# lschoenm/MerKurio

Measured on AMD Instinct MI355X. Metric: Gbases/s scanned (150bp FASTQ, 10k 31-mers); % HBM roofline at 1/2/4/8 GPUs, higher is better.
Workload: dtype u8

## Files before the change

### include/merkurio_hip.h

```cpp
#ifndef MERKURIO_HIP_H
#define MERKURIO_HIP_H

#include <stddef.h>
#include <stdint.h>

#ifdef __cplusplus
extern "C" {
#endif

#define MK_ABI_VERSION 7

#define MK_OK 0
#define MK_E_EMPTY_PATTERN (-1)
#define MK_E_INVALID_Q (-2)
#define MK_E_PATTERN_TOO_LONG (-3)
#define MK_E_NO_PATTERNS (-4)
#define MK_E_NOMEM (-5)
#define MK_E_PAIR_MISMATCH (-6)
#define MK_E_HIP (-7)
#define MK_E_CAPACITY (-8)
#define MK_E_INVALID_ARG (-9)
#define MK_E_UNSUPPORTED (-10)
#define MK_E_RCCL (-11)
#define MK_E_CORRUPT (-12)
// ... 82 lines not shown
#define MK_SUM_RECORDS 2
#define MK_SUM_BASES 3
#define MK_SUM_CANDIDATES 4

int mk_scan_device(mk_matcher *m, const void *d_seq, uint64_t n_bytes, const void *d_seq_off, uint64_t n_rec,
                   uint32_t mode, void *d_rec_flags, void *d_hits, uint64_t hits_cap, void *d_n_hits,
                   void *d_counters, void *stream);

int mk_matcher_check_device(mk_matcher *m, void *stream);

int mk_matcher_hint_hit_density(mk_matcher *m, uint32_t records_hit_per_1000);

int mk_matcher_set_fixed_record_length(mk_matcher *m, uint32_t record_length);

int mk_matcher_hint_record_lengths(mk_matcher *m, int equal_lengths);

int mk_order_hits(const mk_matcher *m, mk_hit *hits, uint64_t n_hits);
int mk_order_hits_device(mk_matcher *m, void *d_hits, uint64_t n_hits, void *stream);
int mk_matcher_order_info(const mk_matcher *m, uint32_t *path, uint32_t *n_bins, uint32_t *max_bin);
int mk_matcher_order_stats(const mk_matcher *m, uint64_t calls[4]);

const char *mk_matcher_kernel_name(const mk_matcher *m);
int mk_matcher_launch_info(const mk_matcher *m, uint32_t *grid_blocks, uint32_t *block_threads, uint32_t *lds_bytes);
int mk_matcher_enable_timing(mk_matcher *m, uint32_t slots);
int mk_matcher_kernel_times(mk_matcher *m, float *ms, uint32_t cap, uint32_t *n_out);

int mk_extract_single(mk_matcher *m, const uint8_t *seq, const uint64_t *off, uint64_t n_rec, int logging,
                      int invert, uint8_t *keep, mk_row *rows, uint64_t rows_cap, uint64_t *n_rows,
                      mk_counters *counters, uint32_t *pattern_hit_counts);
int mk_extract_paired(mk_matcher *m, const uint8_t *seq1, const uint64_t *off1, uint64_t n_rec1,
                      const uint8_t *seq2, const uint64_t *off2, uint64_t n_rec2, int logging, int invert,
                      uint8_t *keep, mk_row *rows, uint64_t rows_cap, uint64_t *n_rows, mk_counters *counters,
                      uint32_t *pattern_hit_counts);
int mk_tag_records(mk_matcher *m, const uint8_t *seq, const uint64_t *off, uint64_t n_rec, int logging,
                   int filter_matching, int invert, uint8_t *keep, mk_row *rows, uint64_t rows_cap, uint64_t *n_rows,
                   mk_counters *counters, uint32_t *pattern_hit_counts, uint64_t *found_off, uint32_t *found_pat,
                   uint64_t found_cap);
int mk_extract_fastq_text(mk_matcher *m, const uint8_t *text, uint64_t n_text, int logging, int invert, uint64_t rec_cap,
                          uint64_t *n_rec, uint64_t *rec_start, uint8_t *keep, mk_row *rows, uint64_t rows_cap, uint64_t *n_rows,
                          mk_counters *counters, uint32_t *pattern_hit_counts, uint32_t *status);
int mk_upload_text_ahead(mk_matcher *m, const uint8_t *text, uint64_t n_text);
int mk_host_alloc(size_t bytes, void **out);
void mk_host_free(void *p);
int mk_matcher_batch_times(const mk_matcher *m, float ms[4]);

int mk_tag_value(const mk_matcher *m, const uint32_t *found_pat, uint64_t n_found, const char *existing, char *out,
// ... 209 lines not shown
```

### merkurio_amd/csrc/matcher.cpp

```cpp
#include <hip/hip_runtime.h>

#include <algorithm>
#include <chrono>
#include <cmath>
#include <cstdarg>
#include <cstdio>
#include <cstdlib>
#include <cstring>
#include <memory>
#include <string>
#include <vector>

#include "host_common.h"
#include "matcher_internal.h"
#include "scan_kernel.h"

namespace mk {

thread_local char g_last_error[512] = "";

int fail(int code, const char *fmt, ...) {
    va_list ap;
    va_start(ap, fmt);
    vsnprintf(g_last_error, sizeof(g_last_error), fmt, ap);
// ... 461 lines not shown
int mk_matcher_filter_info(const mk_matcher *m, uint32_t *q_gram, uint32_t *stride, uint64_t *entries,
                           uint64_t *table_bytes) {
    if (!m) return fail(MK_E_INVALID_ARG, "null matcher");
    if (q_gram) *q_gram = m->q;
    if (stride) *stride = m->S;
    if (entries) *entries = m->entries;
    if (table_bytes) *table_bytes = (uint64_t)m->table_slots * sizeof(TableEntry);
    return MK_OK;
}

int mk_matcher_class_info(const mk_matcher *m, uint32_t *split_len, uint32_t *n_short, uint32_t *q_gram2, uint32_t *stride2) {
    if (!m) return fail(MK_E_INVALID_ARG, "null matcher");
    if (split_len) *split_len = m->split_len;
    if (n_short) *n_short = m->n_short;
    if (q_gram2) *q_gram2 = m->q2;
    if (stride2) *stride2 = m->S2;
    return MK_OK;
}

int mk_matcher_filter_mode(const mk_matcher *m, uint32_t *in_lds, uint64_t *filter_bytes) {
    if (!m) return fail(MK_E_INVALID_ARG, "null matcher");
    if (in_lds) *in_lds = m->gbloom_blocks ? 0 : 1;
    if (filter_bytes) *filter_bytes = m->gbloom_blocks ? (uint64_t)m->gbloom_blocks * 8 : (uint64_t)kBloomBytes;
    return MK_OK;
}

int mk_scan_device(mk_matcher *m, const void *d_seq, uint64_t n_bytes, const void *d_seq_off, uint64_t n_rec,
                   uint32_t mode, void *d_rec_flags, void *d_hits, uint64_t hits_cap, void *d_n_hits,
                   void *d_counters, void *stream) {
    if (!m) return fail(MK_E_INVALID_ARG, "null matcher");
    if (mode > MK_MODE_HITS) return fail(MK_E_INVALID_ARG, "unknown mode %u", mode);
    if (((uintptr_t)d_seq & 15) != 0) return fail(MK_E_INVALID_ARG, "d_seq must be 16-byte aligned");
    if (((uintptr_t)d_rec_flags & 3) != 0) return fail(MK_E_INVALID_ARG, "d_rec_flags must be 4-byte aligned");
    const uint32_t rec_len = m->batch_rec_len ? m->batch_rec_len : m->fixed_rec_len;
    if (rec_len && n_bytes != n_rec * (uint64_t)rec_len)
        return fail(MK_E_INVALID_ARG, "fixed record length %u: %llu records are not %llu bytes", rec_len, (unsigned long long)n_rec,
                    (unsigned long long)n_bytes);
    if (!d_n_hits || !d_rec_flags || (!d_seq_off && n_rec && !rec_len)) return fail(MK_E_INVALID_ARG, "null device buffer");
    if (mode == MK_MODE_HITS && !d_hits && hits_cap) return fail(MK_E_INVALID_ARG, "d_hits is null");
    hipStream_t st = (hipStream_t)stream;
    MK_HIP(hipSetDevice(m->device));
    launch_clear((uint32_t *)d_rec_flags, (n_rec + 3) / 4, (unsigned long long *)d_n_hits, st);
    MK_HIP(hipGetLastError());
    if (mode == MK_MODE_HITS) MK_HIP(hipMemsetAsync(m->d_error, 0, sizeof(uint32_t), st));
    m->last_n_rec = n_rec;
    if (n_rec == 0 || n_bytes == 0) return MK_OK;
// ... 14 lines not shown
    p.n_pat = m->n_pat;
    p.q = m->q;
    const uint64_t kmask = m->q >= 32 ? ~0ull : ((1ull << (2 * m->q)) - 1);
    p.key_mask_lo = (uint32_t)kmask;
    p.key_mask_hi = (uint32_t)(kmask >> 32);
    p.case_insensitive = (m->flags & MK_FLAG_ASCII_CASE_INSENSITIVE) ? 1 : 0;
    p.s2 = m->split_len ? m->S2 : 0;
    p.s2_log2 = m->S2 >= 8 ? 3 : m->S2 >= 4 ? 2 : m->S2 >= 2 ? 1 : 0;
    p.key2_mask = (1u << (2 * m->q2)) - 1u;
    p.short_bytes = m->q2 <= kShortByteMaxQ;
    p.short_bitmap = m->d_short_table;
    p.uniform_len = m->uniform_len;
    p.rec_flags32 = (uint32_t *)d_rec_flags;
    p.hits = (mk_hit *)d_hits;
    p.hits_cap = (mode == MK_MODE_HITS) ? hits_cap : 0;
    p.n_hits = (unsigned long long *)d_n_hits;
    p.counters = (unsigned long long *)d_counters;
    p.error_word = m->d_error;
    const uint64_t waves_per_block = kBlockThreads / 64;
    uint64_t blocks = (n_tiles + waves_per_block - 1) / waves_per_block;
    if (blocks > (uint64_t)m->num_cus) blocks = m->num_cus;
    p.stage = m->d_stage;
    p.rec_per_byte = (double)n_rec / (double)n_bytes;
    const uint64_t tiles_per_wave = n_tiles / (blocks * waves_per_block);
    p.tile_run = m->tile_run ? m->tile_run : tiles_per_wave >= 16 ? 4 : tiles_per_wave >= 8 ? 2 : 1;
    p.rec_index = nullptr;
    p.rec_len = rec_len;
    p.inv_rec_len = rec_len ? 1.0 / (double)rec_len : 0.0;
    if (m->ragged && !rec_len && n_rec < (1ull << 32)) {
        int rc_i = ensure((void **)&m->d_rec_index, &m->d_rec_index_cap, ((n_bytes >> kRecIndexShift) + 2) * sizeof(uint32_t));
        if (rc_i) return rc_i;
        launch_rec_index(p.rec_off, n_rec, n_bytes, m->d_rec_index, st);
        p.rec_index = m->d_rec_index;
    }
    const size_t slots = m->ev_start.size();
    const size_t slot = slots ? (size_t)(m->timed_launches % slots) : 0;
    if (slots) MK_HIP(hipEventRecord(m->ev_start[slot], st));
    const uint32_t kDensePerMille = mode == MK_MODE_HITS ? 95 : 145;
    const bool plain_loads = m->hit_density_pm >= kDensePerMille && !m->split_len;
    const int flavour = plain_loads ? 0 : 1;
    const bool listed = !(plain_loads && m->gbloom_blocks == 0) && mode != MK_MODE_HITS && n_rec < (1ull << 32);
    p.flag_list = listed ? m->d_flag_list : nullptr;
    p.flag_counts = m->d_flag_counts;
    p.flag_cap = kFlagListCap;
    const char *name = launch_scan(p, (int)m->S, m->q > 16, mode == MK_MODE_HITS, m->gbloom_blocks != 0, flavour, (int)blocks, st);
    if (!name) return fail(MK_E_UNSUPPORTED, "no kernel for stride %u", m->S);
    if (slots) {
        MK_HIP(hipEventRecord(m->ev_stop[slot], st));
        m->timed_launches++;
    }
    if (listed)
        launch_flag_scatter(m->d_flag_list, m->d_flag_counts, kFlagListCap, (uint32_t)(blocks * waves_per_block), (uint8_t *)d_rec_flags, st);
    if (d_counters) {
        launch_count_flags(p, st);
        if (mode == MK_MODE_HITS && p.hits && p.hits_cap) launch_hist_hits(p, m->num_cus, st);
    }
    m->kernel_name = name;
    m->last_grid = (int)blocks;
    MK_HIP(hipGetLastError());
    return MK_OK;
}

static int take_device_errors(mk_matcher *m, hipStream_t st) {
    uint32_t w = 0;
    MK_HIP(hipMemcpyAsync(&w, m->d_error, sizeof(w), hipMemcpyDeviceToHost, st));
    MK_HIP(hipStreamSynchronize(st));
    if (!w) return MK_OK;
    MK_HIP(hipMemsetAsync(m->d_error, 0, sizeof(w), st));
    return fail(MK_E_UNSUPPORTED, "an occurrence lies 4 GiB or more into its record: a single record must be shorter than 4 GiB "
                                  "(mk_hit.pos is 32 bits); the tuples of that scan are not usable");
}

int mk_matcher_check_device(mk_matcher *m, void *stream) {
    if (!m) return fail(MK_E_INVALID_ARG, "null matcher");
    MK_HIP(hipSetDevice(m->device));
    return take_device_errors(m, (hipStream_t)stream);
}

int mk_matcher_hint_hit_density(mk_matcher *m, uint32_t records_hit_per_1000) {
    if (!m) return fail(MK_E_INVALID_ARG, "null matcher");
    m->hit_density_pm = records_hit_per_1000 > 1000 ? 1000 : records_hit_per_1000;
// ... 379 lines not shown
```

### merkurio_amd/csrc/matcher_internal.h

```cpp
#pragma once
#include <hip/hip_runtime.h>

#include <mutex>
#include <vector>

#include "filter.hpp"
#include "scan_kernel.h"
#include "host_common.h"

struct mk_matcher {
    int device = 0;
    int num_cus = 256;
    uint32_t algo = MK_ALGO_AC;
    uint32_t flags = 0;
    uint32_t n_pat = 0;
    std::vector<uint8_t> pat_bytes;
    std::vector<uint32_t> pat_off;
    uint32_t uniform_len = 0;
    uint32_t q = 0, S = 1;
    uint32_t split_len = 0, S2 = 0, q2 = 0, n_short = 0;
    uint32_t *d_short_table = nullptr;
    uint64_t entries = 0;
    uint32_t table_slots = 0;
    uint32_t *d_bloom = nullptr;
    uint32_t gbloom_blocks = 0;
    uint32_t tile_run = 0;
    uint32_t hit_density_pm = 0;
    bool ragged = false;
    uint32_t fixed_rec_len = 0, batch_rec_len = 0;
    uint32_t *d_rec_index = nullptr;
// ... 32 lines not shown
        size_t d_text_cap = 0, d_ing_a_cap = 0, d_ing_b_cap = 0, d_fa_seq_cap = 0;
    } txt[2];
    uint32_t bam_piece = 0;
    uint8_t *d_flags2 = nullptr;
    size_t d_flags2_cap = 0;
    void *d_refs = nullptr;
    size_t d_refs_cap = 0;
    std::vector<uint8_t> refs_names;
    std::vector<uint64_t> refs_off;
    uint32_t refs_slots = 0;
    bool refs_valid = false;
    struct AheadSlot {
        void *d = nullptr;
        size_t cap = 0;
        hipEvent_t ev = nullptr;
        const uint8_t *text = nullptr;
        uint64_t n = 0;
    } ahead[4];
    hipStream_t stream_ahead = nullptr;
    std::mutex ahead_mu;
    float batch_ms[4] = {0, 0, 0, 0};
    const char *kernel_name = "";
    int last_grid = 0;
    std::vector<hipEvent_t> ev_start, ev_stop;
    uint64_t timed_launches = 0;
    void *comm = nullptr;
    int comm_rank = 0, comm_size = 0;
};

namespace mk {
int ensure_device(void **p, size_t *cap, size_t need);
extern thread_local double g_alloc_ms, g_free_ms;
int batch_check(const uint8_t *seq_bytes, const uint64_t *seq_off, uint64_t n_rec, uint64_t *n_bytes);
int batch_upload(mk_matcher *m, const uint8_t *seq_bytes, const uint64_t *seq_off, uint64_t n_rec, uint64_t n_bytes, uint32_t *batch_len);
int batch_scan(mk_matcher *m, uint64_t n_bytes, uint64_t n_rec, uint32_t mode, uint32_t batch_len, uint64_t cap, uint64_t limit,
               unsigned long long *found);
int batch_flags(mk_matcher *m, uint64_t n_rec, uint8_t *rec_flags, uint64_t *flagged_out);
int order_hits_on_device(mk_matcher *m, void *d_hits, uint64_t n_hits, bool ac_order, uint64_t rec_bound, void *stream);
int hip_fail(hipError_t e, const char *what);
}
```

### merkurio_amd/csrc/scan_kernel.h

```cpp
#pragma once
#include <hip/hip_runtime.h>
#include <stdint.h>

#include "../../include/merkurio_hip.h"
#include "filter.hpp"

namespace mk {

constexpr uint32_t kHitStage = 1024;
constexpr uint32_t kFlagListCap = 2048;

struct ScanParams {
    const uint8_t *seq;
    uint64_t n_bytes;
    const uint64_t *rec_off;
    uint64_t n_rec;
    const uint32_t *bloom;
    uint32_t gbloom_blocks;
    const TableEntry *table;
    uint32_t table_mask;
    const uint8_t *pat_bytes;
    const uint32_t *pat_off;
    uint32_t n_pat;
    uint32_t q;
    uint32_t key_mask_lo;
    uint32_t key_mask_hi;
    uint32_t s2;
    uint32_t s2_log2;
    uint32_t key2_mask;
    uint32_t short_bytes;
    const uint32_t *short_bitmap;
    uint32_t case_insensitive;
    uint32_t uniform_len;
    double rec_per_byte;
    uint32_t tile_run;
    const uint32_t *rec_index;
    uint32_t rec_len;
    double inv_rec_len;
    mk_hit *stage;
    uint32_t *rec_flags32;
    uint32_t *flag_list;
    uint32_t *flag_counts;
    uint32_t flag_cap;
    mk_hit *hits;
    uint64_t hits_cap;
    unsigned long long *n_hits;
    unsigned long long *counters;
    uint32_t *error_word;
};

const char *launch_scan(const ScanParams &p, int S, bool wide, bool emit, bool global_filter, int flavour, int grid_blocks,
                        hipStream_t stream);

template <int S, int QC, bool EMIT, bool GF, int FL, int MC = 0>
void launch_variant(const ScanParams &p, int grid_blocks, hipStream_t stream);

uint32_t scan_lds_bytes();

// ... 130 lines not shown
```

### merkurio_amd/csrc/scan_kernel_impl.hpp

```cpp
#pragma once
#include <algorithm>

#include "scan_kernel.h"

namespace mk {

typedef uint32_t u32x4 __attribute__((ext_vector_type(4)));

__device__ __forceinline__ uint32_t pack4_top(uint32_t d) { return (d & 0x06060606u) * 0x00820820u; }
__device__ __forceinline__ uint32_t pack16(uint4 v) {
    const uint32_t u0 = pack4_top(v.x), u1 = pack4_top(v.y), u2 = pack4_top(v.z), u3 = pack4_top(v.w);
    const uint32_t lo16 = __builtin_amdgcn_perm(u1, u0, 0x0c0c0703u);
    const uint32_t hi16 = __builtin_amdgcn_perm(u3, u2, 0x07030c0cu);
    return lo16 | hi16;
}

__device__ __forceinline__ uint4 load16(const uint8_t *__restrict__ seq, uint64_t pos, uint64_t n) {
    if (pos + 16 <= n) return *reinterpret_cast<const uint4 *>(seq + pos);
    uint32_t w[4] = {0, 0, 0, 0};
    if (pos < n) {
        uint32_t rem = (uint32_t)(n - pos);
        for (uint32_t i = 0; i < rem; ++i) w[i >> 2] |= (uint32_t)seq[pos + i] << (8 * (i & 3));
    }
    return make_uint4(w[0], w[1], w[2], w[3]);
// ... 352 lines not shown
    if constexpr (!GF) {
        const uint4 *src = reinterpret_cast<const uint4 *>(P.bloom);
        uint4 *dst = reinterpret_cast<uint4 *>(bloom);
        for (uint32_t i = threadIdx.x; i < kBloomWords / 4; i += kBlockThreads) dst[i] = src[i];
    }
    if constexpr (MC != 0) {
        const uint4 *src2 = reinterpret_cast<const uint4 *>(P.short_bitmap);
        uint4 *dst2 = reinterpret_cast<uint4 *>(lds_all);
        for (uint32_t i = threadIdx.x; i < kShortBitmapWords / 4; i += kBlockThreads) dst2[i] = src2[i];
    }
    if constexpr (!GF || MC != 0) __syncthreads();
    const uint2 *__restrict__ gbloom = reinterpret_cast<const uint2 *>(P.bloom);
    const uint32_t gmask = P.gbloom_blocks;

    if (P.counters && blockIdx.x == 0 && threadIdx.x == 0) {
        atomicAdd(&P.counters[P.n_pat + MK_SUM_RECORDS], (unsigned long long)P.n_rec);
        atomicAdd(&P.counters[P.n_pat + MK_SUM_BASES], (unsigned long long)P.n_bytes);
    }
    const uint32_t lane = threadIdx.x & 63u;
    const uint32_t wave_in_block = __builtin_amdgcn_readfirstlane(threadIdx.x >> 6);
    const uint64_t wave_id = (uint64_t)blockIdx.x * (kBlockThreads / 64) + wave_in_block;
    const uint64_t n_waves = (uint64_t)gridDim.x * (kBlockThreads / 64);
    constexpr int NS = G::kNS;
    constexpr uint64_t kTileBytes = (uint64_t)kTileChunks * kChunkBytes;
    const uint32_t mask_lo = P.key_mask_lo, mask_hi = P.key_mask_hi;
    const uint8_t *__restrict__ seq = P.seq;
    const uint64_t n_bytes = P.n_bytes;
    CandEntry *ring = reinterpret_cast<CandEntry *>(bloom + kBloomWords) + wave_in_block * kRingEntries;
    uint32_t *ctx_ring = bloom + wave_in_block * kRingEntries;
    uint32_t q_head = 0, q_count = 0, n_cand = 0;
    HitRing hr;
    hr.q = reinterpret_cast<uint2 *>(bloom + kBloomWords + (kBlockThreads / 64) * kRingEntries * 2) + wave_in_block * kHitSlots;
    hr.count = 0;
    hr.stage = EMIT ? P.stage + wave_id * (uint64_t)kHitStage : nullptr;
    hr.staged = 0;
    hr.flist = (!kWide && !EMIT && P.flag_list) ? P.flag_list + wave_id * (uint64_t)P.flag_cap : nullptr;
    hr.nflag = 0;
    uint32_t n_true = 0;
    uint32_t abl_acc = 0;

    auto halo = [&](uint32_t pk_cur, uint32_t pk_nxt, uint32_t &w1, uint32_t &w2) __attribute__((always_inline)) {
        w1 = 0;
        w2 = 0;
        if constexpr (G::kNeedW1) {
            const uint32_t n0 = __builtin_amdgcn_readlane(pk_nxt, 0);
            w1 = __builtin_amdgcn_update_dpp(n0, pk_cur, 0x130, 0xf, 0xf, false);
        }
// ... 140 lines not shown
                    const uint32_t khi = __builtin_amdgcn_alignbit(w2, w1, sh) & mask_hi;
                    const uint32_t t = __builtin_amdgcn_alignbit(khi, klo, 24);
                    slot_h = __umul24(klo, 0x9E3779u) + __umul24(t, 0x85EBCBu) + (t & 0xFF000000u);
                }
                if constexpr (kCtx) {
                    const uint32_t pb = 2u * j * S;
                    const uint32_t prev7 = pb >= 14u ? (w0 >> (pb - 14u)) : __builtin_amdgcn_alignbit(w0, wm1, (pb + 18u) & 31u);
                    const uint32_t next7 = stream32_rt(w0, w1, w2, pb + 2u * (uint32_t)QC);
                    slot_c = (prev7 & 0x3FFFu) | ((next7 & 0x3FFFu) << 14);
                }
                slot_t = t_base + j * S;
                if constexpr (MC != 0) {
                    const uint32_t j2 = (j - 16u) << P.s2_log2;
                    const uint32_t fp2 = short_fp(__builtin_amdgcn_alignbit(w1, w0, 2u * j2) & P.key2_mask);
                    const bool is2 = j >= 16u;
                    slot_h = is2 ? fp2 : main_fp(slot_h);
                    slot_t = is2 ? t_base + j2 : slot_t;
                }
                slot_full = true;
            }
        } while (__ballot(cand != 0));
    };

    const uint64_t n_main_tiles = n_bytes >= kChunkBytes ? (n_bytes - kChunkBytes) / kTileBytes : 0;
    if (wave_id * (P.tile_run ? P.tile_run : 1u) < n_main_tiles) {
        const uint32_t run = P.tile_run ? P.tile_run : 1u;
        const uint64_t jump = (n_waves - 1) * (uint64_t)run + 1;
        uint64_t ld_tile = wave_id * run;
        uint32_t ld_run = 0;
        uint32_t ld_g = 0;
        const uint64_t last_tile = n_main_tiles - 1;
        const uint8_t *ld_ptr = seq + (ld_tile < last_tile ? ld_tile : last_tile) * kTileBytes + lane * 16;
        auto nt_load = [](const uint8_t *p) -> uint4 {
            if constexpr (NTL) {
                const u32x4 nv = __builtin_nontemporal_load(reinterpret_cast<const u32x4 *>(p));
                return make_uint4(nv.x, nv.y, nv.z, nv.w);
            } else {
                return *reinterpret_cast<const uint4 *>(p);
            }
        };
        auto load_group = [&](uint4 &a, uint4 &b, uint4 &c, uint4 &d) __attribute__((always_inline)) {
            a = nt_load(ld_ptr);
            b = nt_load(ld_ptr + kChunkBytes);
            c = nt_load(ld_ptr + 2 * kChunkBytes);
            d = nt_load(ld_ptr + 3 * kChunkBytes);
            ld_ptr += 4 * kChunkBytes;
            if (++ld_g == (uint32_t)(kTileChunks + 1) / 4) {
                ld_g = 0;
                if (++ld_run == run) {
                    ld_run = 0;
                    ld_tile += jump;
                } else {
                    ld_tile += 1;
                }
                const uint64_t t = ld_tile < last_tile ? ld_tile : last_tile;
                ld_ptr = seq + t * kTileBytes + lane * 16;
            }
        };
        uint4 r0, r1, r2, r3;
        load_group(r0, r1, r2, r3);
        uint32_t pk_prev = 0;
        uint32_t pk_pp = 0, pk_tile_prev = 0;
        bool pd_on = false;
        uint32_t pd_h0 = 0, pd_h1 = 0, pd_cur = 0, pd_nxt = 0, pd_wm1 = 0;
        uint2 pd_b0 = make_uint2(0, 0), pd_b1 = pd_b0;
        uint64_t pd_cpos = 0;
        auto test_pending = [&]() __attribute__((always_inline)) {
            auto pass = [](uint32_t h, uint2 blk) -> uint32_t {
                const uint32_t hb = gbloom_bits(h);
                return (blk.x >> (hb >> 27)) & (blk.x >> (hb >> 12)) & (blk.y >> (hb >> 22)) & (blk.y >> (hb >> 17)) & 1u;
            };
            uint32_t cand = pass(pd_h0, pd_b0);
            if constexpr (NS > 1) cand |= pass(pd_h1, pd_b1) << 1;
            if (__ballot(cand != 0)) queue_candidates(pd_cur, pd_nxt, pd_wm1, cand, pd_cpos, pd_h0, pd_h1);
        };
        uint64_t last_push_base = 0;
        uint32_t sc_run = 0;
        for (uint64_t tile = wave_id * run; tile < n_main_tiles;) {
            const uint64_t base = tile * kTileBytes;
            if constexpr (kCtx) {
                pk_tile_prev = 0;
                if (base >= 16) pk_tile_prev = pack16(*reinterpret_cast<const uint4 *>(seq + base - 16));
            }
            if (base - last_push_base >= (1ull << 30)) {
                last_push_base = base;
                flush_slots();
                if (hr.count) drain_hits<EMIT, FL>(P, hr, newest_end, lane, n_true);
                if (q_count && !pend_on) issue_probe(q_count < 64 ? q_count : 64);
            }
#pragma unroll 1
            for (int g = 0; g < (kTileChunks + 1) / 4; ++g) {
                const uint32_t p0 = pack16(r0), p1 = pack16(r1), p2 = pack16(r2), p3 = pack16(r3);
                asm volatile("" ::"v"(p0), "v"(p1), "v"(p2), "v"(p3) : "memory");
                if (pend_on) consume_probe();
                load_group(r0, r1, r2, r3);
                {
                    uint32_t q0 = p0, q1 = p1, q2 = p2;
#pragma unroll 1
                    for (int k = 0; k < 4; ++k) {
                        const int ci = 4 * g + k - 1;
                        if constexpr (kPipe) {
                            uint32_t nh0 = 0, nh1 = 0, nwm1 = 0;
                            uint2 nb0 = make_uint2(0, 0), nb1 = nb0;
                            if (ci >= 0) {
                                uint32_t w1, w2;
                                halo(pk_prev, q0, w1, w2);
                                nh0 = sample_hash<S, QC>(pk_prev, w1, w2, 0, mask_lo, mask_hi);
                                nb0 = gbloom[gbloom_block(nh0, gmask)];
                                if constexpr (NS > 1) {
                                    nh1 = sample_hash<S, QC>(pk_prev, w1, w2, 2 * S, mask_lo, mask_hi);
                                    nb1 = gbloom[gbloom_block(nh1, gmask)];
                                }
                                nwm1 = __builtin_amdgcn_update_dpp(__builtin_amdgcn_readlane(pk_pp, 63), pk_prev, 0x138, 0xf, 0xf, false);
                            }
// ... 18 lines not shown
                                queue_candidates(pk_prev, q0, wm1, ck, base + (uint64_t)ci * kChunkBytes, h0, h1);
                            }
                        }
                        if constexpr (kCtx) pk_pp = ci < 0 ? pk_tile_prev : pk_prev;
                        pk_prev = q0;
                        q0 = q1;
                        q1 = q2;
                        q2 = p3;
                    }
                }
                if constexpr ((MK_ABLATE & 8) != 0) {
                    if (q_count >= MK_ISSUE_AT) {
                        q_head = (q_head + q_count) & (kRingEntries - 1);
                        q_count = 0;
                    }
                } else if (!pend_on && q_count >= (FL == 0 ? MK_ISSUE_AT_DENSE : MK_ISSUE_AT)) {
                    issue_probe(q_count < 64 ? q_count : 64);
                }
                if constexpr (FL == 0 && MK_DRAIN_AT_DENSE <= 64) {
                    if (hr.count >= MK_DRAIN_AT_DENSE) drain_hits<EMIT, FL>(P, hr, newest_end, lane, n_true);
                }
                pk_prev = p3;
            }
            if (++sc_run == run) {
                sc_run = 0;
                tile += jump;
            } else {
                tile += 1;
            }
        }
        if constexpr (kPipe) {
            if (pd_on) test_pending();
        }
    }
    if (pend_on) consume_probe();

    {
        const uint64_t tail_rank = (wave_id + n_waves - (n_main_tiles / (P.tile_run ? P.tile_run : 1u)) % n_waves) % n_waves;
        for (uint64_t cpos = n_main_tiles * kTileBytes + tail_rank * kChunkBytes; cpos < n_bytes; cpos += n_waves * kChunkBytes) {
            const uint32_t pk_cur = pack16(load16(seq, cpos + lane * 16, n_bytes));
            const uint32_t pk_nxt = pack16(load16(seq, cpos + kChunkBytes + lane * 16, n_bytes));
            uint32_t h0 = 0, h1 = 0;
            const uint32_t ck = filter_chunk(pk_cur, pk_nxt, h0, h1);
            if constexpr ((MK_ABLATE & 4) != 0) n_cand += ck;
            if (__ballot(ck != 0)) {
                uint32_t wm1 = 0;
                if constexpr (kCtx) {
                    const uint64_t mine = cpos + lane * 16;
                    if (mine >= 16) wm1 = pack16(load16(seq, mine - 16, n_bytes));
                }
                queue_candidates(pk_cur, pk_nxt, wm1, ck, cpos, h0, h1);
            }
        }
    }

    flush_slots();
    while (q_count) drain_ring(q_count < 64 ? q_count : 64);
    if (hr.count) drain_hits<EMIT, FL>(P, hr, newest_end, lane, n_true);
    if constexpr (EMIT) flush_stage<!kWide>(P, hr, lane);
    if (hr.flist && lane == 0) P.flag_counts[wave_id] = hr.nflag;
    if ((MK_ABLATE & 1) != 0 && abl_acc == 0xFFFFFFFFu) n_cand++;
    if (P.counters) {
// ... 13 lines not shown
```

### merkurio_amd/native.py

```python
import ctypes as C
import time
import importlib.util
import os

import numpy as np

from . import build as _build

MK_OK = 0
MK_E_EMPTY_PATTERN = -1
MK_E_INVALID_Q = -2
MK_E_PATTERN_TOO_LONG = -3
MK_E_NO_PATTERNS = -4
MK_E_NOMEM = -5
MK_E_PAIR_MISMATCH = -6
MK_E_HIP = -7
MK_E_CAPACITY = -8
MK_E_INVALID_ARG = -9
MK_E_UNSUPPORTED = -10
MK_E_RCCL = -11
MK_E_CORRUPT = -12
MK_COMM_ID_BYTES = 128

MK_ALGO_AUTO, MK_ALGO_AC, MK_ALGO_BNDMQ = 0, 1, 2
MK_FLAG_ASCII_CASE_INSENSITIVE = 1
MK_MODE_ANY, MK_MODE_HITS = 0, 1
MK_NUM_SUMMARY = 8
MK_SUM_HITS, MK_SUM_RECORDS_HIT, MK_SUM_RECORDS, MK_SUM_BASES, MK_SUM_CANDIDATES = 0, 1, 2, 3, 4

HIT_DTYPE = np.dtype([("rec", "<u8"), ("pat", "<u4"), ("pos", "<u4")])
ROW_DTYPE = np.dtype([("rec", "<u8"), ("pat", "<u4"), ("pos", "<u4"), ("file", "<u4"), ("_pad", "<u4")])

EXPORTS = [
    "mk_abi_version", "mk_last_error", "mk_device_count", "mk_read_kmers_from_text", "mk_parse_pattern_list",
    "mk_reverse_complement", "mk_canonical", "mk_recommend_aho_corasick", "mk_tune_q_value", "mk_generate_masks",
    "mk_free", "mk_matcher_create", "mk_matcher_create_ex", "mk_plan_geometry", "mk_matcher_destroy", "mk_matcher_algo", "mk_matcher_num_patterns",
    "mk_matcher_filter_info", "mk_matcher_class_info", "mk_matcher_filter_mode", "mk_scan_batch", "mk_scan_device", "mk_order_hits", "mk_order_hits_device", "mk_matcher_order_info", "mk_matcher_order_stats", "mk_matcher_kernel_name",
    "mk_matcher_launch_info", "mk_matcher_enable_timing", "mk_matcher_kernel_times", "mk_matcher_hint_hit_density", "mk_matcher_hint_record_lengths", "mk_matcher_set_fixed_record_length", "mk_matcher_check_device",
    "mk_extract_single", "mk_extract_fastq_text", "mk_upload_text_ahead", "mk_host_alloc", "mk_host_free", "mk_extract_paired", "mk_tag_records", "mk_tag_value", "mk_matcher_batch_times", "mk_synth_reads_device",
    "mk_synth_reads_host", "mk_synth_reads_device_range", "mk_reduce_counters", "mk_reduce_prepare", "mk_comm_available", "mk_comm_unique_id", "mk_comm_init",
    "mk_comm_reduce_counters", "mk_comm_size", "mk_comm_destroy",
    "mk_codec_create", "mk_codec_destroy", "mk_bgzf_deflate_bound", "mk_bgzf_deflate", "mk_bgzf_deflate_pieces", "mk_bgzf_inflate", "mk_bgzf_members", "mk_bgzf_eof",
    "mk_codec_times", "mk_codec_set_pass_limits", "mk_codec_set_inflate_kernel", "mk_codec_set_gzip_chunk", "mk_gzip_inflate_device", "mk_gzip_text_read", "mk_gzip_text_device", "mk_gzip_text_release", "mk_gzip_info", "mk_extract_fastq_bgzf", "mk_extract_window",
    "mk_tag_bam_window", "mk_matcher_set_bam_piece", "mk_tag_sam_window", "mk_tag_sam_bam_window", "mk_tag_bam_sam_window",
]


class MerkurioError(RuntimeError):
    def __init__(self, code, msg):
        super().__init__(f"[{code}] {msg}")
        self.code = code


class PatternError(MerkurioError):
    KINDS = {MK_E_EMPTY_PATTERN: "EmptyPattern", MK_E_INVALID_Q: "InvalidQGramLength",
             MK_E_PATTERN_TOO_LONG: "PatternTooLong"}

    @property
    def kind(self):
        return self.KINDS.get(self.code, "?")


class MatcherOptions(C.Structure):
    _fields_ = [("struct_size", C.c_uint32), ("force_stride", C.c_uint32), ("force_global_filter", C.c_uint32),
                ("gbloom_log2_blocks", C.c_uint32), ("tile_run", C.c_uint32), ("gbloom_kib", C.c_uint32),
                ("length_classes", C.c_uint32), ("force_split_len", C.c_uint32), ("force_stride2", C.c_uint32),
                ("force_q2", C.c_uint32)]

    def __init__(self, force_stride=0, force_global_filter=False, gbloom_log2_blocks=0, tile_run=0, gbloom_kib=0,
                 length_classes=0, force_split_len=0, force_stride2=0, force_q2=0, force_single_class=False):
        super().__init__(C.sizeof(MatcherOptions), int(force_stride), int(bool(force_global_filter)),
                         int(gbloom_log2_blocks), int(tile_run), int(gbloom_kib),
                         1 if force_single_class else int(length_classes), int(force_split_len), int(force_stride2), int(force_q2))


class WindowText(C.Structure):
    _fields_ = [("text", C.c_void_p), ("text_cap", C.c_uint64), ("tail", C.c_void_p), ("tail_cap", C.c_uint64), ("kept", C.c_void_p),
                ("kept_cap", C.c_uint64), ("n_text", C.c_uint64), ("n_used", C.c_uint64), ("n_tail", C.c_uint64), ("n_kept_bytes", C.c_uint64)]


class WindowSource(C.Structure):
    _fields_ = [("head", C.c_void_p), ("n_head", C.c_uint64), ("text", C.c_void_p), ("n_text", C.c_uint64), ("bgzf", C.c_void_p),
                ("n_bgzf", C.c_uint64), ("members", C.c_void_p), ("n_members", C.c_uint64), ("device_text", C.c_void_p), ("n_device_text", C.c_uint64), ("ends_at_record", C.c_uint32),
                ("reserved", C.c_uint32), ("rec_start", C.c_void_p), ("tail", C.c_void_p), ("tail_cap", C.c_uint64), ("kept", C.c_void_p),
                ("kept_cap", C.c_uint64), ("all", C.c_void_p), ("all_cap", C.c_uint64), ("n_window", C.c_uint64), ("n_used", C.c_uint64),
                ("n_tail", C.c_uint64), ("n_kept_bytes", C.c_uint64), ("n_rec_seen", C.c_uint64)]


MK_TEXT_FASTQ, MK_TEXT_FASTA = 0, 1


class BamWindow(C.Structure):
    _fields_ = [("head", C.c_void_p), ("n_head", C.c_uint64), ("bgzf", C.c_void_p), ("n_bgzf", C.c_uint64), ("members", C.c_void_p), ("n_members", C.c_uint64),
                ("last", C.c_uint32), ("filter_matching", C.c_uint32), ("invert", C.c_uint32), ("tag", C.c_uint8 * 2), ("reserved", C.c_uint8 * 2),
                ("block_bytes", C.c_uint32), ("tail", C.c_void_p), ("tail_cap", C.c_uint64), ("out", C.c_void_p), ("out_cap", C.c_uint64),
                ("rows", C.c_void_p), ("rows_cap", C.c_uint64), ("row_name", C.c_void_p), ("names", C.c_void_p), ("names_cap", C.c_uint64),
# ... 90 lines not shown
    L.mk_matcher_num_patterns.argtypes = [C.c_void_p]
    L.mk_matcher_num_patterns.restype = C.c_uint32
    L.mk_matcher_create.argtypes = [C.c_void_p, C.c_void_p, C.c_uint32, C.c_uint32, C.c_uint32, C.c_uint32, C.c_int32,
                                    C.POINTER(C.c_void_p)]
    L.mk_matcher_create_ex.argtypes = [C.c_void_p, C.c_void_p, C.c_uint32, C.c_uint32, C.c_uint32, C.c_uint32, C.c_int32,
                                       C.POINTER(MatcherOptions), C.POINTER(C.c_void_p)]
    L.mk_synth_reads_device_range.argtypes = [C.c_void_p, C.c_uint64, C.c_uint64, C.c_uint64, C.c_uint32, C.c_uint32,
                                              C.c_void_p, C.c_void_p, C.c_void_p]
    L.mk_reduce_counters.argtypes = [C.POINTER(C.c_void_p), C.c_int, C.POINTER(C.c_void_p), C.c_size_t, C.c_void_p]
    L.mk_reduce_prepare.argtypes = [C.POINTER(C.c_void_p), C.c_int]
    L.mk_comm_unique_id.argtypes = [C.c_void_p]
    L.mk_comm_init.argtypes = [C.c_void_p, C.c_void_p, C.c_int, C.c_int]
    L.mk_comm_reduce_counters.argtypes = [C.c_void_p, C.c_void_p, C.c_size_t, C.c_void_p]
    L.mk_comm_destroy.argtypes = [C.c_void_p]
    L.mk_comm_size.argtypes = [C.c_void_p, C.POINTER(C.c_int)]
    L.mk_scan_batch.argtypes = [C.c_void_p, C.c_void_p, C.c_void_p, C.c_uint64, C.c_uint32, C.c_void_p, C.c_void_p,
                                C.c_uint64, C.POINTER(C.c_uint64)]
    L.mk_scan_device.argtypes = [C.c_void_p, C.c_void_p, C.c_uint64, C.c_void_p, C.c_uint64, C.c_uint32, C.c_void_p,
                                 C.c_void_p, C.c_uint64, C.c_void_p, C.c_void_p, C.c_void_p]
    L.mk_order_hits.argtypes = [C.c_void_p, C.c_void_p, C.c_uint64]
    L.mk_order_hits_device.argtypes = [C.c_void_p, C.c_void_p, C.c_uint64, C.c_void_p]
    L.mk_matcher_order_info.argtypes = [C.c_void_p, C.POINTER(C.c_uint32), C.POINTER(C.c_uint32), C.POINTER(C.c_uint32)]
    L.mk_matcher_launch_info.argtypes = [C.c_void_p, C.POINTER(C.c_uint32), C.POINTER(C.c_uint32), C.POINTER(C.c_uint32)]
    L.mk_matcher_enable_timing.argtypes = [C.c_void_p, C.c_uint32]
    L.mk_matcher_hint_hit_density.argtypes = [C.c_void_p, C.c_uint32]
    L.mk_matcher_hint_record_lengths.argtypes = [C.c_void_p, C.c_int]
    L.mk_matcher_set_fixed_record_length.argtypes = [C.c_void_p, C.c_uint32]
    L.mk_matcher_check_device.argtypes = [C.c_void_p, C.c_void_p]
    L.mk_matcher_batch_times.argtypes = [C.c_void_p, C.POINTER(C.c_float)]
    L.mk_matcher_kernel_times.argtypes = [C.c_void_p, C.c_void_p, C.c_uint32, C.POINTER(C.c_uint32)]
    L.mk_matcher_filter_info.argtypes = [C.c_void_p, C.POINTER(C.c_uint32), C.POINTER(C.c_uint32),
                                         C.POINTER(C.c_uint64), C.POINTER(C.c_uint64)]
    L.mk_matcher_filter_mode.argtypes = [C.c_void_p, C.POINTER(C.c_uint32), C.POINTER(C.c_uint64)]
    L.mk_plan_geometry.argtypes = [C.c_void_p, C.c_uint32, C.POINTER(MatcherOptions)] + [C.POINTER(C.c_uint32)] * 7
    L.mk_matcher_class_info.argtypes = [C.c_void_p, C.POINTER(C.c_uint32), C.POINTER(C.c_uint32), C.POINTER(C.c_uint32),
                                        C.POINTER(C.c_uint32)]
    L.mk_extract_single.argtypes = [C.c_void_p, C.c_void_p, C.c_void_p, C.c_uint64, C.c_int, C.c_int, C.c_void_p,
                                    C.c_void_p, C.c_uint64, C.POINTER(C.c_uint64), C.POINTER(Counters), C.c_void_p]
    L.mk_extract_fastq_text.argtypes = [C.c_void_p, C.c_void_p, C.c_uint64, C.c_int, C.c_int, C.c_uint64, C.POINTER(C.c_uint64), C.c_void_p,
                                        C.c_void_p, C.c_void_p, C.c_uint64, C.POINTER(C.c_uint64), C.POINTER(Counters), C.c_void_p,
                                        C.POINTER(C.c_uint32)]
    L.mk_upload_text_ahead.argtypes = [C.c_void_p, C.c_void_p, C.c_uint64]
    L.mk_host_alloc.argtypes = [C.c_size_t, C.POINTER(C.c_void_p)]
    L.mk_host_free.argtypes = [C.c_void_p]
    L.mk_host_free.restype = None
    L.mk_codec_create.argtypes = [C.c_int, C.POINTER(C.c_void_p)]
# ... 142 lines not shown
    q = load().mk_tune_q_value(len(pattern))
    if q == 0:
        raise MerkurioError(MK_E_PATTERN_TOO_LONG, "Pattern length is too long for BNDMq.")
    return q


def generate_masks(pattern: bytes):
    src = np.frombuffer(bytes(pattern) + b"\0", dtype=np.uint8)
    masks = np.zeros(256, dtype=np.uint64)
    accept = C.c_uint64()
    _check(load().mk_generate_masks(src.ctypes.data, len(pattern), masks.ctypes.data, C.byref(accept)))
    return masks.tolist(), accept.value


def plan_geometry(lengths, options=None):
    lens = np.ascontiguousarray(lengths, dtype=np.uint32)
    opt = None if options is None else (options if isinstance(options, MatcherOptions) else MatcherOptions(**options))
    v = [C.c_uint32() for _ in range(7)]
    _check(load().mk_plan_geometry(lens.ctypes.data, len(lens), None if opt is None else C.byref(opt), *[C.byref(x) for x in v]))
    keys = ("q_gram", "stride", "in_lds", "split_len", "n_short", "q_gram2", "stride2")
    return dict(zip(keys, (x.value for x in v)))


class Matcher:

    def __init__(self, patterns, algo=MK_ALGO_AUTO, q=0, case_insensitive=False, device=0, options=None):
        self.patterns = [p.encode() if isinstance(p, str) else bytes(p) for p in patterns]
        data, off = pack_list(self.patterns)
        self._h = C.c_void_p()
        flags = MK_FLAG_ASCII_CASE_INSENSITIVE if case_insensitive else 0
        if options is None:
            _check(load().mk_matcher_create(data.ctypes.data, off.ctypes.data, len(self.patterns), algo, q, flags,
                                            device, C.byref(self._h)))
        else:
            opt = options if isinstance(options, MatcherOptions) else MatcherOptions(**options)
            _check(load().mk_matcher_create_ex(data.ctypes.data, off.ctypes.data, len(self.patterns), algo, q, flags,
                                               device, C.byref(opt), C.byref(self._h)))
        self.device = device

    def close(self):
        if getattr(self, "_h", None):
            load().mk_matcher_destroy(self._h)
            self._h = None

    def __del__(self):
        try:
# ... 1 lines not shown
        except Exception:
            pass

    @property
    def handle(self):
        return self._h

    @property
    def algo(self):
        return load().mk_matcher_algo(self._h)

    @property
    def use_ac(self):
        return self.algo == MK_ALGO_AC

    @property
    def kernel_name(self):
        return load().mk_matcher_kernel_name(self._h).decode()

    def launch_info(self):
        g, b, l = C.c_uint32(), C.c_uint32(), C.c_uint32()
        _check(load().mk_matcher_launch_info(self._h, C.byref(g), C.byref(b), C.byref(l)))
        return {"grid_blocks": g.value, "block_threads": b.value, "lds_bytes": l.value}

    def batch_times_ms(self):
        ms = (C.c_float * 4)()
        _check(load().mk_matcher_batch_times(self._h, ms))
        return {"upload": ms[0], "device": ms[1], "download": ms[2], "host": ms[3]}

    def order_info(self):
        a, b, c = C.c_uint32(), C.c_uint32(), C.c_uint32()
        _check(load().mk_matcher_order_info(self._h, C.byref(a), C.byref(b), C.byref(c)))
        return {"path": a.value, "bins": b.value, "max_bin": c.value}

    def enable_timing(self, slots):
        _check(load().mk_matcher_enable_timing(self._h, slots))
        self._timing_slots = slots

    def kernel_times_ms(self):
        cap = max(1, getattr(self, "_timing_slots", 0))
        ms = np.zeros(cap, dtype=np.float32)
        n = C.c_uint32()
        _check(load().mk_matcher_kernel_times(self._h, ms.ctypes.data, cap, C.byref(n)))
        return ms[:n.value].tolist()

    def filter_info(self):
# ... 508 lines not shown
```

Before: 6217.

## Replace tile runs with long contiguous tiles and balanced short-tile remainder geometry

Each wave now scans one long contiguous tile per run, merged from several short tiles so the overlap chunk is not reloaded, instead of a sequence of separate adjacent tiles. The remaining bytes are split into short tiles whose size is chosen to balance loads across waves. The old run-jump bookkeeping in the loader and scan loops is removed and a run of 8 is added for large inputs. This reduces redundant halo loads and tail imbalance, at the cost of per-tile base and group computation, possibly fewer blocks, and a new geometry-inspection API.

```diff
diff --git a/include/merkurio_hip.h b/include/merkurio_hip.h
--- a/include/merkurio_hip.h
+++ b/include/merkurio_hip.h
@@ -128,6 +128,17 @@
 
 const char *mk_matcher_kernel_name(const mk_matcher *m);
 int mk_matcher_launch_info(const mk_matcher *m, uint32_t *grid_blocks, uint32_t *block_threads, uint32_t *lds_bytes);
+typedef struct {
+    uint64_t n_waves;
+    uint64_t n_long_tiles, long_tile_bytes;
+    uint64_t n_short_tiles, short_tile_bytes;
+    uint64_t tail_start;
+    uint32_t long_tile_loads, short_tile_loads;
+    uint32_t tile_run;
+    uint32_t reserved;
+} mk_tile_geometry;
+int mk_scan_tile_geometry(uint64_t n_bytes, uint64_t n_waves, uint32_t tile_run, mk_tile_geometry *out);
+int mk_matcher_scan_geometry(const mk_matcher *m, mk_tile_geometry *out);
 int mk_matcher_enable_timing(mk_matcher *m, uint32_t slots);
 int mk_matcher_kernel_times(mk_matcher *m, float *ms, uint32_t cap, uint32_t *n_out);
 
diff --git a/merkurio_amd/csrc/matcher.cpp b/merkurio_amd/csrc/matcher.cpp
--- a/merkurio_amd/csrc/matcher.cpp
+++ b/merkurio_amd/csrc/matcher.cpp
@@ -507,6 +507,34 @@
     if (!m) return fail(MK_E_INVALID_ARG, "null matcher");
     if (in_lds) *in_lds = m->gbloom_blocks ? 0 : 1;
     if (filter_bytes) *filter_bytes = m->gbloom_blocks ? (uint64_t)m->gbloom_blocks * 8 : (uint64_t)kBloomBytes;
+    return MK_OK;
+}
+
+static void export_geometry(const TileGeometry &g, uint64_t n_waves, uint32_t run, mk_tile_geometry *out) {
+    out->n_waves = n_waves;
+    out->n_long_tiles = g.n_long;
+    out->long_tile_bytes = g.long_bytes;
+    out->n_short_tiles = g.n_short;
+    out->short_tile_bytes = g.short_bytes;
+    out->tail_start = g.tail_start;
+    out->long_tile_loads = g.long_loads;
+    out->short_tile_loads = g.short_loads;
+    out->tile_run = run;
+    out->reserved = 0;
+}
+
+int mk_scan_tile_geometry(uint64_t n_bytes, uint64_t n_waves, uint32_t tile_run, mk_tile_geometry *out) {
+    if (!out) return fail(MK_E_INVALID_ARG, "null geometry");
+    if (n_waves == 0 || tile_run > kMaxTileRun)
+        return fail(MK_E_INVALID_ARG, "tile geometry: %llu waves, tile_run %u (0..8)", (unsigned long long)n_waves, tile_run);
+    if (tile_run == 0) tile_run = tile_run_rule(n_bytes, n_waves);
+    export_geometry(tile_geometry(n_bytes, n_waves, tile_run), n_waves, tile_run, out);
+    return MK_OK;
+}
+
+int mk_matcher_scan_geometry(const mk_matcher *m, mk_tile_geometry *out) {
+    if (!m || !out) return fail(MK_E_INVALID_ARG, "null argument");
+    export_geometry(m->last_geo, (uint64_t)m->last_grid * (kBlockThreads / 64), m->last_run, out);
     return MK_OK;
 }
 
@@ -567,8 +595,18 @@
     if (blocks > (uint64_t)m->num_cus) blocks = m->num_cus;
     p.stage = m->d_stage;
     p.rec_per_byte = (double)n_rec / (double)n_bytes;
-    const uint64_t tiles_per_wave = n_tiles / (blocks * waves_per_block);
-    p.tile_run = m->tile_run ? m->tile_run : tiles_per_wave >= 16 ? 4 : tiles_per_wave >= 8 ? 2 : 1;
+    uint32_t run = m->tile_run ? m->tile_run : tile_run_rule(n_bytes, blocks * waves_per_block);
+    while (run > 1 && blocks * waves_per_block * ((uint64_t)(run * (kTileChunks + 1) - 1) * kChunkBytes) > (1ull << 30)) --run;
+    if (run > 1 && blocks < (uint64_t)m->num_cus) {
+        const uint64_t long_bytes = (uint64_t)(run * (kTileChunks + 1) - 1) * kChunkBytes;
+        blocks = std::min<uint64_t>(blocks, std::max<uint64_t>(1, n_bytes / (long_bytes * waves_per_block)));
+    }
+    const TileGeometry geo = tile_geometry(n_bytes, blocks * waves_per_block, run);
+    p.n_long_tiles = geo.n_long;
+    p.n_tiles = geo.n_long + geo.n_short;
+    p.tail_start = geo.tail_start;
+    p.long_groups = geo.long_loads / 4;
+    p.short_groups = geo.short_loads / 4;
     p.rec_index = nullptr;
     p.rec_len = rec_len;
     p.inv_rec_len = rec_len ? 1.0 / (double)rec_len : 0.0;
@@ -602,6 +640,8 @@
     }
     m->kernel_name = name;
     m->last_grid = (int)blocks;
+    m->last_geo = geo;
+    m->last_run = run;
     MK_HIP(hipGetLastError());
     return MK_OK;
 }
diff --git a/merkurio_amd/csrc/matcher_internal.h b/merkurio_amd/csrc/matcher_internal.h
--- a/merkurio_amd/csrc/matcher_internal.h
+++ b/merkurio_amd/csrc/matcher_internal.h
@@ -6,6 +6,7 @@
 
 #include "filter.hpp"
 #include "scan_kernel.h"
+#include "tile_geometry.hpp"
 #include "host_common.h"
 
 struct mk_matcher {
@@ -84,6 +85,8 @@
     float batch_ms[4] = {0, 0, 0, 0};
     const char *kernel_name = "";
     int last_grid = 0;
+    mk::TileGeometry last_geo{};
+    uint32_t last_run = 0;
     std::vector<hipEvent_t> ev_start, ev_stop;
     uint64_t timed_launches = 0;
     void *comm = nullptr;
diff --git a/merkurio_amd/csrc/scan_kernel.h b/merkurio_amd/csrc/scan_kernel.h
--- a/merkurio_amd/csrc/scan_kernel.h
+++ b/merkurio_amd/csrc/scan_kernel.h
@@ -33,7 +33,8 @@
     uint32_t case_insensitive;
     uint32_t uniform_len;
     double rec_per_byte;
-    uint32_t tile_run;
+    uint64_t n_long_tiles, n_tiles, tail_start;
+    uint32_t long_groups, short_groups;
     const uint32_t *rec_index;
     uint32_t rec_len;
     double inv_rec_len;
diff --git a/merkurio_amd/csrc/scan_kernel_impl.hpp b/merkurio_amd/csrc/scan_kernel_impl.hpp
--- a/merkurio_amd/csrc/scan_kernel_impl.hpp
+++ b/merkurio_amd/csrc/scan_kernel_impl.hpp
@@ -398,7 +398,6 @@
     const uint64_t wave_id = (uint64_t)blockIdx.x * (kBlockThreads / 64) + wave_in_block;
     const uint64_t n_waves = (uint64_t)gridDim.x * (kBlockThreads / 64);
     constexpr int NS = G::kNS;
-    constexpr uint64_t kTileBytes = (uint64_t)kTileChunks * kChunkBytes;
     const uint32_t mask_lo = P.key_mask_lo, mask_hi = P.key_mask_hi;
     const uint8_t *__restrict__ seq = P.seq;
     const uint64_t n_bytes = P.n_bytes;
@@ -585,15 +584,24 @@
         } while (__ballot(cand != 0));
     };
 
-    const uint64_t n_main_tiles = n_bytes >= kChunkBytes ? (n_bytes - kChunkBytes) / kTileBytes : 0;
-    if (wave_id * (P.tile_run ? P.tile_run : 1u) < n_main_tiles) {
-        const uint32_t run = P.tile_run ? P.tile_run : 1u;
-        const uint64_t jump = (n_waves - 1) * (uint64_t)run + 1;
-        uint64_t ld_tile = wave_id * run;
-        uint32_t ld_run = 0;
+    const uint64_t n_main_tiles = P.n_tiles;
+    const uint64_t n_long_tiles = P.n_long_tiles;
+    const uint32_t long_groups = P.long_groups;
+    const uint32_t short_groups = P.short_groups;
+    const uint64_t long_bytes = (uint64_t)(4u * long_groups - 1u) * kChunkBytes;
+    const uint64_t short_bytes = (uint64_t)(4u * short_groups - 1u) * kChunkBytes;
+    auto tile_base = [&](uint64_t t) __attribute__((always_inline)) -> uint64_t {
+        return t < n_long_tiles ? t * long_bytes : n_long_tiles * long_bytes + (t - n_long_tiles) * short_bytes;
+    };
+    auto tile_groups = [&](uint64_t t) __attribute__((always_inline)) -> uint32_t {
+        return t < n_long_tiles ? long_groups : short_groups;
+    };
+    if (wave_id < n_main_tiles) {
+        uint64_t ld_tile = wave_id;
         uint32_t ld_g = 0;
+        uint32_t ld_groups = tile_groups(ld_tile);
         const uint64_t last_tile = n_main_tiles - 1;
-        const uint8_t *ld_ptr = seq + (ld_tile < last_tile ? ld_tile : last_tile) * kTileBytes + lane * 16;
+        const uint8_t *ld_ptr = seq + tile_base(ld_tile) + lane * 16;
         auto nt_load = [](const uint8_t *p) -> uint4 {
             if constexpr (NTL) {
                 const u32x4 nv = __builtin_nontemporal_load(reinterpret_cast<const u32x4 *>(p));
@@ -608,16 +616,12 @@
             c = nt_load(ld_ptr + 2 * kChunkBytes);
             d = nt_load(ld_ptr + 3 * kChunkBytes);
             ld_ptr += 4 * kChunkBytes;
-            if (++ld_g == (uint32_t)(kTileChunks + 1) / 4) {
+            if (++ld_g == ld_groups) {
                 ld_g = 0;
-                if (++ld_run == run) {
-                    ld_run = 0;
-                    ld_tile += jump;
-                } else {
-                    ld_tile += 1;
-                }
+                ld_tile += n_waves;
                 const uint64_t t = ld_tile < last_tile ? ld_tile : last_tile;
-                ld_ptr = seq + t * kTileBytes + lane * 16;
+                ld_groups = tile_groups(t);
+                ld_ptr = seq + tile_base(t) + lane * 16;
             }
         };
         uint4 r0, r1, r2, r3;
@@ -638,9 +642,9 @@
             if (__ballot(cand != 0)) queue_candidates(pd_cur, pd_nxt, pd_wm1, cand, pd_cpos, pd_h0, pd_h1);
         };
         uint64_t last_push_base = 0;
-        uint32_t sc_run = 0;
-        for (uint64_t tile = wave_id * run; tile < n_main_tiles;) {
-            const uint64_t base = tile * kTileBytes;
+        for (uint64_t tile = wave_id; tile < n_main_tiles; tile += n_waves) {
+            const uint64_t base = tile_base(tile);
+            const int groups = (int)tile_groups(tile);
             if constexpr (kCtx) {
                 pk_tile_prev = 0;
                 if (base >= 16) pk_tile_prev = pack16(*reinterpret_cast<const uint4 *>(seq + base - 16));
@@ -652,7 +656,7 @@
                 if (q_count && !pend_on) issue_probe(q_count < 64 ? q_count : 64);
             }
 #pragma unroll 1
-            for (int g = 0; g < (kTileChunks + 1) / 4; ++g) {
+            for (int g = 0; g < groups; ++g) {
                 const uint32_t p0 = pack16(r0), p1 = pack16(r1), p2 = pack16(r2), p3 = pack16(r3);
                 asm volatile("" ::"v"(p0), "v"(p1), "v"(p2), "v"(p3) : "memory");
                 if (pend_on) consume_probe();
@@ -717,12 +721,6 @@
                 }
                 pk_prev = p3;
             }
-            if (++sc_run == run) {
-                sc_run = 0;
-                tile += jump;
-            } else {
-                tile += 1;
-            }
         }
         if constexpr (kPipe) {
             if (pd_on) test_pending();
@@ -731,8 +729,8 @@
     if (pend_on) consume_probe();
 
     {
-        const uint64_t tail_rank = (wave_id + n_waves - (n_main_tiles / (P.tile_run ? P.tile_run : 1u)) % n_waves) % n_waves;
-        for (uint64_t cpos = n_main_tiles * kTileBytes + tail_rank * kChunkBytes; cpos < n_bytes; cpos += n_waves * kChunkBytes) {
+        const uint64_t tail_rank = (wave_id + n_waves - n_main_tiles % n_waves) % n_waves;
+        for (uint64_t cpos = P.tail_start + tail_rank * kChunkBytes; cpos < n_bytes; cpos += n_waves * kChunkBytes) {
             const uint32_t pk_cur = pack16(load16(seq, cpos + lane * 16, n_bytes));
             const uint32_t pk_nxt = pack16(load16(seq, cpos + kChunkBytes + lane * 16, n_bytes));
             uint32_t h0 = 0, h1 = 0;
diff --git a/merkurio_amd/csrc/tile_geometry.hpp b/merkurio_amd/csrc/tile_geometry.hpp
--- /dev/null
+++ b/merkurio_amd/csrc/tile_geometry.hpp
@@ -0,0 +1,51 @@
+#pragma once
+#include <stdint.h>
+
+#include "filter.hpp"
+
+namespace mk {
+
+struct TileGeometry {
+    uint64_t n_long, long_bytes;
+    uint64_t n_short, short_bytes;
+    uint64_t tail_start;
+    uint32_t long_loads, short_loads;
+};
+
+constexpr uint32_t kMaxTileRun = 8;
+
+MK_HD uint32_t tile_run_rule(uint64_t n_bytes, uint64_t n_waves) {
+    const uint64_t tile_bytes = (uint64_t)kTileChunks * kChunkBytes;
+    const uint64_t tiles_per_wave = n_waves ? (n_bytes + tile_bytes - 1) / tile_bytes / n_waves : 0;
+    return tiles_per_wave >= 32 ? 8 : tiles_per_wave >= 16 ? 4 : tiles_per_wave >= 8 ? 2 : 1;
+}
+
+MK_HD TileGeometry tile_geometry(uint64_t n_bytes, uint64_t n_waves, uint32_t run) {
+    TileGeometry g{};
+    if (run < 1) run = 1;
+    g.short_bytes = (uint64_t)kTileChunks * kChunkBytes;
+    g.short_loads = (uint32_t)kTileChunks + 1;
+    g.long_loads = run * g.short_loads;
+    g.long_bytes = (uint64_t)(g.long_loads - 1) * kChunkBytes;
+    const uint64_t n_main_tiles = n_bytes >= (uint64_t)kChunkBytes ? (n_bytes - kChunkBytes) / g.short_bytes : 0;
+    if (run > 1 && n_waves) g.n_long = n_main_tiles * g.short_bytes / (n_waves * g.long_bytes) * n_waves;
+    const uint64_t long_end = g.n_long * g.long_bytes;
+    const uint64_t rest = n_bytes >= (uint64_t)kChunkBytes ? n_bytes - kChunkBytes - long_end : 0;
+    if (g.n_long) {
+        uint64_t best = ~0ull;
+        for (uint32_t k = g.short_loads / 4; k >= 4; --k) {
+            const uint64_t tiles = rest / ((uint64_t)(4 * k - 1) * kChunkBytes);
+            const uint64_t loads = (tiles + n_waves - 1) / n_waves * (4 * k);
+            if (loads < best) {
+                best = loads;
+                g.short_loads = 4 * k;
+            }
+        }
+        g.short_bytes = (uint64_t)(g.short_loads - 1) * kChunkBytes;
+    }
+    g.n_short = rest / g.short_bytes;
+    g.tail_start = long_end + g.n_short * g.short_bytes;
+    return g;
+}
+
+}
diff --git a/merkurio_amd/native.py b/merkurio_amd/native.py
--- a/merkurio_amd/native.py
+++ b/merkurio_amd/native.py
@@ -36,7 +36,7 @@
     "mk_reverse_complement", "mk_canonical", "mk_recommend_aho_corasick", "mk_tune_q_value", "mk_generate_masks",
     "mk_free", "mk_matcher_create", "mk_matcher_create_ex", "mk_plan_geometry", "mk_matcher_destroy", "mk_matcher_algo", "mk_matcher_num_patterns",
     "mk_matcher_filter_info", "mk_matcher_class_info", "mk_matcher_filter_mode", "mk_scan_batch", "mk_scan_device", "mk_order_hits", "mk_order_hits_device", "mk_matcher_order_info", "mk_matcher_order_stats", "mk_matcher_kernel_name",
-    "mk_matcher_launch_info", "mk_matcher_enable_timing", "mk_matcher_kernel_times", "mk_matcher_hint_hit_density", "mk_matcher_hint_record_lengths", "mk_matcher_set_fixed_record_length", "mk_matcher_check_device",
+    "mk_matcher_launch_info", "mk_scan_tile_geometry", "mk_matcher_scan_geometry", "mk_matcher_enable_timing", "mk_matcher_kernel_times", "mk_matcher_hint_hit_density", "mk_matcher_hint_record_lengths", "mk_matcher_set_fixed_record_length", "mk_matcher_check_device",
     "mk_extract_single", "mk_extract_fastq_text", "mk_upload_text_ahead", "mk_host_alloc", "mk_host_free", "mk_extract_paired", "mk_tag_records", "mk_tag_value", "mk_matcher_batch_times", "mk_synth_reads_device",
     "mk_synth_reads_host", "mk_synth_reads_device_range", "mk_reduce_counters", "mk_reduce_prepare", "mk_comm_available", "mk_comm_unique_id", "mk_comm_init",
     "mk_comm_reduce_counters", "mk_comm_size", "mk_comm_destroy",
@@ -72,6 +72,15 @@
         super().__init__(C.sizeof(MatcherOptions), int(force_stride), int(bool(force_global_filter)),
                          int(gbloom_log2_blocks), int(tile_run), int(gbloom_kib),
                          1 if force_single_class else int(length_classes), int(force_split_len), int(force_stride2), int(force_q2))
+
+
+class TileGeometry(C.Structure):
+    _fields_ = [("n_waves", C.c_uint64), ("n_long_tiles", C.c_uint64), ("long_tile_bytes", C.c_uint64), ("n_short_tiles", C.c_uint64),
+                ("short_tile_bytes", C.c_uint64), ("tail_start", C.c_uint64), ("long_tile_loads", C.c_uint32),
+                ("short_tile_loads", C.c_uint32), ("tile_run", C.c_uint32), ("reserved", C.c_uint32)]
+
+    def as_dict(self):
+        return {k: int(getattr(self, k)) for k, _ in self._fields_ if k != "reserved"}
 
 
 class WindowText(C.Structure):
@@ -208,6 +217,8 @@
     L.mk_order_hits_device.argtypes = [C.c_void_p, C.c_void_p, C.c_uint64, C.c_void_p]
     L.mk_matcher_order_info.argtypes = [C.c_void_p, C.POINTER(C.c_uint32), C.POINTER(C.c_uint32), C.POINTER(C.c_uint32)]
     L.mk_matcher_launch_info.argtypes = [C.c_void_p, C.POINTER(C.c_uint32), C.POINTER(C.c_uint32), C.POINTER(C.c_uint32)]
+    L.mk_scan_tile_geometry.argtypes = [C.c_uint64, C.c_uint64, C.c_uint32, C.POINTER(TileGeometry)]
+    L.mk_matcher_scan_geometry.argtypes = [C.c_void_p, C.POINTER(TileGeometry)]
     L.mk_matcher_enable_timing.argtypes = [C.c_void_p, C.c_uint32]
     L.mk_matcher_hint_hit_density.argtypes = [C.c_void_p, C.c_uint32]
     L.mk_matcher_hint_record_lengths.argtypes = [C.c_void_p, C.c_int]
@@ -396,6 +407,12 @@
     return dict(zip(keys, (x.value for x in v)))
 
 
+def scan_tile_geometry(n_bytes, n_waves, tile_run):
+    g = TileGeometry()
+    _check(load().mk_scan_tile_geometry(int(n_bytes), int(n_waves), int(tile_run), C.byref(g)))
+    return g.as_dict()
+
+
 class Matcher:
 
     def __init__(self, patterns, algo=MK_ALGO_AUTO, q=0, case_insensitive=False, device=0, options=None):
@@ -443,6 +460,11 @@
         g, b, l = C.c_uint32(), C.c_uint32(), C.c_uint32()
         _check(load().mk_matcher_launch_info(self._h, C.byref(g), C.byref(b), C.byref(l)))
         return {"grid_blocks": g.value, "block_threads": b.value, "lds_bytes": l.value}
+
+    def scan_geometry(self):
+        g = TileGeometry()
+        _check(load().mk_matcher_scan_geometry(self._h, C.byref(g)))
+        return g.as_dict()
 
     def batch_times_ms(self):
         ms = (C.c_float * 4)()
```

Measured after the change: 6335, median of 6. 1.9% higher.
